# Dasch0/nenbody

Hardware: AMD Instinct MI355X
Metric: body-updates/sec (N x steps/s) at N=131072, all-pairs gravity + Euler step (higher is better)
Workload: dtype f32

## Files before the change

### nenbody_amd/csrc/nb_api.hip

```cpp
#include <hip/hip_runtime.h>
#include <dlfcn.h>

#include <cmath>
#include <cstdlib>
#include <algorithm>
#include <atomic>
#include <chrono>
#include <cstring>
#include <mutex>
#include <new>
#include <string>
#include <thread>
#include <vector>

#include "../../include/nenbody.h"
#include "../../include/nenbody_diag.h"
#include "nb_kernels.h"
#include "nb_eyes.h"
#include "nb_frame.h"
#define NB_SRGB_TABLE static const
#define NB_SRGB_WANT_DECODE
#include "nb_srgb_tables.h"
#undef NB_SRGB_WANT_DECODE
#undef NB_SRGB_TABLE

#define NB_EXPORT extern "C" __attribute__((visibility("default")))

namespace {

thread_local std::string g_tls_error = "";

constexpr uint32_t kTargetWaves = 16384;
constexpr uint32_t kMaxSlices = 64;

struct Knob {
    bool set = false;
    uint32_t v = 0;
    uint32_t or_else(uint32_t dflt) const { return set ? v : dflt; }
    bool on() const { return set && v != 0; }
};
struct DebugOverrides {
    Knob tile, fast_pairs_w, fast_pairs_np, fast_pairs_chunk, fast_ib, fast_groups, fast_waves, fast_slices, fast_no_share, strict_force_ieee, force_3d, strict_no_packed, strict_lanes, strict_unroll,
        strict_pc, strict_bc, strict_sl, fast_sl, fast_pairs, ring, ring_np, ring_ga, ring_wpb, ring_c4_own, ring_c4_rest, ring_cap, inst_device_libm, boids_slices, bc_spin_budget, bc_prio, boids_pc, boids_tile, boids_force, selftest_control, roctx, dropin_zero_copy, dropin_poll, dropin_poll_budget_us;
    uint32_t generation = 0;
};

Knob read_knob(const char *name)
{
    Knob k;
    const char *s = std::getenv(name);
    if (s && *s) {
        k.set = true;
        k.v = (uint32_t)std::strtoul(s, nullptr, 10);
    }
    return k;
}

std::atomic<const DebugOverrides *> g_overrides{nullptr};
std::atomic<bool> g_env_enabled{false};
std::atomic<bool> g_rccl_solo{false};
std::mutex g_overrides_mu;

const DebugOverrides *parse_overrides(uint32_t generation)
{
    DebugOverrides *d = new DebugOverrides();
    d->generation = generation;
    d->roctx = read_knob("NB_ROCTX");
    if (!g_env_enabled.load(std::memory_order_relaxed)) return d;
    d->tile = read_knob("NB_TILE");
    d->fast_ib = read_knob("NB_FAST_IB");
    d->fast_groups = read_knob("NB_FAST_GROUPS");
    d->fast_waves = read_knob("NB_FAST_WAVES");
    d->fast_slices = read_knob("NB_FAST_SLICES");
    d->fast_no_share = read_knob("NB_FAST_NO_SHARE");
    d->strict_force_ieee = read_knob("NB_STRICT_FORCE_IEEE");
    d->force_3d = read_knob("NB_FORCE_3D");
    d->strict_no_packed = read_knob("NB_STRICT_NO_PACKED");
    d->strict_lanes = read_knob("NB_STRICT_LANES");
    d->strict_unroll = read_knob("NB_STRICT_UNROLL");
    d->strict_pc = read_knob("NB_STRICT_PC");
    d->strict_bc = read_knob("NB_STRICT_BC");
    d->strict_sl = read_knob("NB_STRICT_SL");
    d->fast_sl = read_knob("NB_FAST_SL");
    d->fast_pairs = read_knob("NB_FAST_PAIRS");
    d->fast_pairs_w = read_knob("NB_FAST_PAIRS_W");
    d->fast_pairs_chunk = read_knob("NB_FAST_PAIRS_CHUNK");
    d->fast_pairs_np = read_knob("NB_FAST_PAIRS_NP");
    d->inst_device_libm = read_knob("NB_INST_DEVICE_LIBM");
    d->ring = read_knob("NB_RING");
    d->ring_np = read_knob("NB_RING_NP");
    d->ring_ga = read_knob("NB_RING_GA");
    d->ring_wpb = read_knob("NB_RING_WPB");
    d->ring_c4_own = read_knob("NB_RING_C4_OWN");
    d->ring_c4_rest = read_knob("NB_RING_C4_REST");
    d->ring_cap = read_knob("NB_RING_CAP");
    d->bc_spin_budget = read_knob("NB_BC_SPIN_BUDGET");
    d->bc_prio = read_knob("NB_BC_PRIO");
    d->boids_pc = read_knob("NB_BOIDS_PC");
    d->boids_tile = read_knob("NB_BOIDS_TILE");
    d->boids_force = read_knob("NB_BOIDS_FORCE");
    d->boids_slices = read_knob("NB_BOIDS_SLICES");
    d->dropin_zero_copy = read_knob("NB_DROPIN_ZERO_COPY");
    d->dropin_poll = read_knob("NB_DROPIN_POLL");
    d->dropin_poll_budget_us = read_knob("NB_DROPIN_POLL_BUDGET_US");
    d->selftest_control = read_knob("NB_SELFTEST_CONTROL");
    return d;
}

const DebugOverrides &overrides()
{
    const DebugOverrides *d = g_overrides.load(std::memory_order_acquire);
    if (d) return *d;
    std::lock_guard<std::mutex> lock(g_overrides_mu);
    d = g_overrides.load(std::memory_order_acquire);
    if (!d) {
        d = parse_overrides(1);
        g_overrides.store(d, std::memory_order_release);
    }
    return *d;
}

bool valid_tile(uint32_t t) { return t == 256 || t == 512 || t == 1024; }

struct Plan {
    uint32_t tile;
    uint32_t ib;
    uint32_t waves;
    uint32_t groups;
    uint32_t slices;
    uint32_t j_chunk;
    uint32_t lo_bits, hi_bits, force_ieee;
    int guard_a, guard_b, guard_g, guard_c;
    uint32_t force_3d;
    uint32_t unroll;
    uint32_t lanes;
    uint32_t pc;
    uint32_t no_packed;
    uint32_t bc;
    uint32_t pairs;
    uint32_t pairs_np;
    uint32_t pairs_chunk;
    uint32_t fsl;
    uint32_t sl;
    uint32_t spin_budget;
    uint32_t bc_prio;
    uint32_t n_total;
};

int floor_log2f(float x)
{
    int e;
    std::frexp(x, &e);
    return e - 1;
}

uint32_t fast_bodies_per_lane(uint32_t n_total, uint32_t count)
{
    const uint64_t pairs = (uint64_t)n_total * count;
    uint32_t ib = overrides().fast_ib.or_else(pairs >= (1ull << 31) ? 4u : pairs >= (1ull << 27) ? 2u : 1u);
    return (ib == 1 || ib == 2 || ib == 4) ? ib : 1u;
}

uint32_t fast_wave_form()
{
    const uint32_t w = overrides().fast_waves.or_else(8u);
    return (w == 1 || w == 4 || w == 8 || w == 16) ? w : 0u;
}

void fast_split(uint32_t n_fold, uint32_t count, uint32_t ib, uint32_t waves, uint32_t *tile, uint32_t *groups, uint32_t *slices,
                uint32_t *chunk)
{
    const DebugOverrides &dbg = overrides();
    if (waves && *tile == 1024u) *tile = 512u;
    if (waves && *tile == 512u && (ib == 1 || waves == 1)) *tile = 256u;
    const uint32_t bodies = waves ? 64u * ib : 256u * ib, chunk_waves = waves ? 1u : 4u;
    const uint32_t blocks = (count + bodies - 1u) / bodies;
    const uint32_t max_by_tiles = std::max(1u, (n_fold + *tile - 1u) / *tile);
    uint32_t split = (kTargetWaves + blocks * chunk_waves - 1u) / (blocks * chunk_waves);
    if (split > max_by_tiles) split = max_by_tiles;
    if (split < 1) split = 1;
    uint32_t g = waves ? waves : dbg.fast_groups.or_else(split >= 4u ? 4u : split >= 2u ? 2u : 1u);
    if (!waves && g != 1 && g != 2 && g != 4) g = 1;
    if (!waves && *tile == 1024u) g = 1;
    uint32_t sl = dbg.fast_slices.or_else((split + g - 1u) / g);
    if (sl > kMaxSlices) sl = kMaxSlices;
    if (sl < 1) sl = 1;
    uint32_t chunks = sl * g;
    if (chunks > max_by_tiles) chunks = max_by_tiles;
    uint32_t c = (std::max(n_fold, 1u) + chunks - 1u) / chunks;
    c = ((c + *tile - 1u) / *tile) * *tile;
    chunks = (std::max(n_fold, 1u) + c - 1u) / c;
    sl = (chunks + g - 1u) / g;
    *groups = g;
    *slices = sl;
    *chunk = c;
}

int make_plan(const nb_params &p, uint32_t n_total, uint32_t count, Plan *out, std::string *err)
{
    if (n_total == 0 || count == 0 || count > n_total) {
        *err = "nb: need 0 < count <= n_total";
        return NB_ERR_INVALID;
    }
    if (p.mode != NB_MODE_STRICT && p.mode != NB_MODE_FAST) {
        *err = "nb: params.mode must be NB_MODE_STRICT or NB_MODE_FAST";
        return NB_ERR_INVALID;
    }
    if (n_total > 0x80000000u) {
        *err = "nb: sets of more than 2^31 bodies are not supported";
        return NB_ERR_UNSUPPORTED;
    }
    const DebugOverrides &dbg = overrides();
    Plan pl{};
    pl.tile = p.tile;
    if (pl.tile == 0) pl.tile = dbg.tile.or_else((p.mode == NB_MODE_STRICT) ? 1024u : fast_wave_form() ? 256u : 512u);
    if (!valid_tile(pl.tile)) {
        *err = "nb: params.tile must be 0, 256, 512 or 1024";
        return NB_ERR_INVALID;
    }
    pl.ib = 1;
    pl.groups = 1;
    pl.slices = 1;
    pl.j_chunk = n_total;
    if (p.mode == NB_MODE_FAST) {
        pl.ib = fast_bodies_per_lane(n_total, count);
        pl.waves = fast_wave_form();
        fast_split(n_total, count, pl.ib, pl.waves, &pl.tile, &pl.groups, &pl.slices, &pl.j_chunk);
    }
    if (p.mode == NB_MODE_FAST) {
        const bool no_form_named = p.tile == 0 && !dbg.tile.set && !dbg.fast_waves.set && !dbg.fast_groups.set;
        pl.fsl = dbg.fast_sl.or_else((pl.waves == 8u && n_total >= 4096u && no_form_named) ? 1u : 0u);
        constexpr uint32_t kPairsMinN = 32768u;
        const bool pairs_ok = count == n_total && n_total % 256u == 0 && n_total <= 4194304u;
        uint32_t pnp = (n_total >= 98304u && n_total % 512u == 0) ? 4u : 2u;
        if (dbg.fast_pairs_np.set && (dbg.fast_pairs_np.v == 2 || (dbg.fast_pairs_np.v == 4 && n_total % 512u == 0))) pnp = dbg.fast_pairs_np.v;
        uint32_t pw = pnp == 4u ? (n_total >= 131072u ? 4u : 2u) : (n_total >= 131072u ? 8u : 4u);
        if (dbg.fast_pairs_w.set && (dbg.fast_pairs_w.v == 1 || dbg.fast_pairs_w.v == 2 || dbg.fast_pairs_w.v == 4 || (dbg.fast_pairs_w.v == 8 && pnp == 2u)))
            pw = dbg.fast_pairs_w.v;
        pl.pairs = (pairs_ok && dbg.fast_pairs.or_else((n_total >= kPairsMinN && no_form_named && !dbg.fast_sl.set && !dbg.fast_ib.set &&
                                                        !dbg.fast_slices.set) ? 1u : 0u)) ? pw : 0u;
        pl.pairs_np = pnp;
        pl.pairs_chunk = 0;
        if (pl.pairs && dbg.fast_pairs_chunk.on()) {
            const uint32_t super = 128u * pnp * pw;
            pl.pairs_chunk = std::max(super, dbg.fast_pairs_chunk.v / super * super);
        }
        if (pl.pairs) pl.fsl = 0;
        if (pl.fsl) {
            uint32_t tile = 256u;
            pl.waves = 8u;
            fast_split(n_total, count, pl.ib, pl.waves, &tile, &pl.groups, &pl.slices, &pl.j_chunk);
            pl.tile = tile;
        }
    }
    pl.force_ieee = 1;
    pl.lo_bits = 0x3f800000u;
    pl.hi_bits = 0x3f800000u;
    const float G = std::fabs(p.G);
    if (std::isfinite(p.G) && std::isfinite(p.bias) && G > 0.f && p.bias > 0.f) {
        const int g = floor_log2f(G), c = floor_log2f(p.bias);
        const int b = 20;
        const int dmax = std::max(2 * b + 4, c + 2);
        int a = std::max(-100 + 23 - g, -120 + 23 - g + dmax);
        const bool ok = g >= -100 && g <= 100 && c >= -100 && dmax <= 100 && (b + 2 + g - c) <= 120 && a <= b - 1;
        if (ok) {
            if (a < -120) a = -120;
            pl.lo_bits = (uint32_t)(a + 127) << 23;
            pl.hi_bits = (uint32_t)(b + 127) << 23;
            pl.force_ieee = 0;
            pl.guard_a = a;
            pl.guard_b = b;
            pl.guard_g = g;
            pl.guard_c = c;
        }
    }
    if (dbg.strict_force_ieee.on()) pl.force_ieee = 1;
    if (p.mode == NB_MODE_FAST) {
        const bool bias_ok = std::isfinite(p.bias) && p.bias >= 0x1p-60f && p.bias <= 0x1p60f;
        pl.force_ieee = (!bias_ok || dbg.fast_no_share.on()) ? 1u : 0u;
    }
    pl.force_3d = dbg.force_3d.on() ? 2u : 0u;
    pl.no_packed = dbg.strict_no_packed.on() ? 1u : 0u;
    constexpr uint32_t kChainMax = 57344u;
    pl.lanes = 1;
    if (count <= kChainMax)
        while (pl.lanes < 16 && (uint64_t)count * pl.lanes < 2048ull * 64ull) pl.lanes *= 2;
    pl.lanes = dbg.strict_lanes.or_else(pl.lanes);
    if (pl.lanes != 1 && pl.lanes != 2 && pl.lanes != 4 && pl.lanes != 8 && pl.lanes != 16) pl.lanes = 1;
    pl.unroll = dbg.strict_unroll.or_else(pl.lanes == 1 ? 8 : (pl.lanes == 16 ? 2 : 4));
    if (pl.lanes == 1 && pl.unroll != 4 && pl.unroll != 8 && pl.unroll != 16) pl.unroll = 8;
    if (pl.lanes > 1 && pl.unroll != 2 && pl.unroll != 4) pl.unroll = 4;
    if (pl.lanes == 16) pl.unroll = 2;
    if (p.mode == NB_MODE_STRICT && pl.lanes > 1 && pl.tile == 512) pl.tile = 1024;
    if (p.mode == NB_MODE_STRICT && pl.lanes > 1 && pl.tile == 1024 && pl.unroll == 2 && pl.lanes < 8) pl.unroll = 4;
    constexpr uint32_t kSmallSet = 1536u;
    pl.pc = dbg.strict_pc.or_else((count <= kChainMax && n_total >= kSmallSet) ? 14u : 0u);
    if (pl.pc == 1) pl.pc = 8;
    if (pl.pc != 0 && pl.pc != 8 && pl.pc != 14) pl.pc = 8;
    pl.n_total = n_total;
    pl.bc = dbg.strict_bc.or_else((count <= kChainMax && n_total >= kSmallSet && !dbg.strict_pc.set && !dbg.strict_lanes.set) ? 1u : 0u);
    pl.bc = (pl.bc && p.mode == NB_MODE_STRICT) ? 1u : 0u;
    pl.spin_budget = dbg.bc_spin_budget.or_else(0u);
    pl.bc_prio = dbg.bc_prio.or_else(1u) ? 1u : 0u;
    pl.sl = dbg.strict_sl.or_else((!pl.bc && !pl.pc && pl.lanes == 1 && p.tile == 0 && !dbg.tile.set && !dbg.strict_lanes.set &&
                                   !dbg.strict_pc.set && !dbg.strict_unroll.set && !dbg.strict_no_packed.set && n_total >= kSmallSet) ? 1u : 0u);
    pl.sl = (pl.sl && p.mode == NB_MODE_STRICT && !pl.bc) ? std::min(pl.sl, 3u) : 0u;
    *out = pl;
    return NB_OK;
}

size_t plan_scratch_bytes(const Plan &pl, uint32_t count)
{
    if (pl.bc || pl.sl) return nbk::strict_bc_scratch_bytes(pl.n_total);
    if (pl.pairs) return nbk::strict_bc_scratch_bytes(pl.n_total) + nbk::fast_pairs_scratch_floats(pl.n_total, pl.pairs, pl.pairs_np, pl.pairs_chunk) * sizeof(float);
    if (pl.fsl) return nbk::strict_bc_scratch_bytes(pl.n_total) + (pl.slices > 1 ? (size_t)pl.slices * count * sizeof(float4) : 0);
    return pl.slices > 1 ? (size_t)pl.slices * count * sizeof(float4) : 0;
}

int cached_plan(const nb_params &p, uint32_t n_total, uint32_t count, const Plan **out, std::string *err)
{
    struct Entry {
        bool valid = false;
        nb_params p{};
        uint32_t n_total = 0, count = 0, generation = 0;
        Plan pl{};
    };
    constexpr int kEntries = 4;
    thread_local Entry cache[kEntries];
    thread_local int next = 0;
    const uint32_t gen = overrides().generation;
    for (int i = 0; i < kEntries; ++i) {
        const Entry &e = cache[i];
        if (e.valid && e.n_total == n_total && e.count == count && e.generation == gen && std::memcmp(&e.p, &p, sizeof(p)) == 0) {
            *out = &e.pl;
            return NB_OK;
        }
    }
    Plan pl;
    int rc = make_plan(p, n_total, count, &pl, err);
    if (rc != NB_OK) return rc;
    Entry &e = cache[next];
    next = (next + 1) % kEntries;
    e.valid = true;
    e.p = p;
    e.n_total = n_total;
    e.count = count;
    e.generation = gen;
    e.pl = pl;
    *out = &e.pl;
    return NB_OK;
}

struct Roctx {
    int (*push)(const char *) = nullptr;
    int (*pop)() = nullptr;
};
const Roctx *roctx_api()
{
    if (!overrides().roctx.on()) return nullptr;
    static const Roctx *api = [] {
        Roctx *r = new Roctx();
        void *h = dlopen("librocprofiler-sdk-roctx.so.1", RTLD_NOW | RTLD_LOCAL);
        if (!h) h = dlopen("librocprofiler-sdk-roctx.so", RTLD_NOW | RTLD_LOCAL);
        if (!h) h = dlopen("libroctx64.so.4", RTLD_NOW | RTLD_LOCAL);
        if (!h) h = dlopen("libroctx64.so", RTLD_NOW | RTLD_LOCAL);
        if (h) {
            r->push = (int (*)(const char *))dlsym(h, "roctxRangePushA");
            r->pop = (int (*)())dlsym(h, "roctxRangePop");
        }
        return (const Roctx *)r;
    }();
    return (api->push && api->pop) ? api : nullptr;
}
struct RoctxRange {
    const Roctx *api;
    explicit RoctxRange(const char *name) : api(roctx_api())
    {
        if (api) (void)api->push(name);
    }
    ~RoctxRange()
    {
        if (api) (void)api->pop();
    }
    RoctxRange(const RoctxRange &) = delete;
    RoctxRange &operator=(const RoctxRange &) = delete;
};

constexpr int kMaxDevices = 64;
uint32_t *g_status_word[kMaxDevices] = {};
std::mutex g_status_mu;

int device_status_word(uint32_t **out, std::string *err)
{
    int dev = 0;
    hipError_t e = hipGetDevice(&dev);
    if (e != hipSuccess || dev < 0 || dev >= kMaxDevices) {
        *err = std::string("nb: hipGetDevice failed: ") + hipGetErrorString(e);
        return NB_ERR_HIP;
    }
    std::lock_guard<std::mutex> lock(g_status_mu);
    if (!g_status_word[dev]) {
        uint32_t *w = nullptr;
        e = hipMalloc((void **)&w, 64);
        if (e == hipSuccess) e = hipMemset(w, 0, 64);
        if (e != hipSuccess) {
            *err = std::string("nb: allocating the device status word failed: ") + hipGetErrorString(e);
            return e == hipErrorOutOfMemory ? NB_ERR_ALLOC : NB_ERR_HIP;
        }
        g_status_word[dev] = w;
    }
    *out = g_status_word[dev];
    return NB_OK;
}

int check_status_word(uint32_t *w, std::string *err)
{
    if (!w) return NB_OK;
    uint32_t v = 0;
    hipError_t e = hipMemcpy(&v, w, sizeof(v), hipMemcpyDeviceToHost);
    if (e != hipSuccess) {
        *err = std::string("nb: reading the device status word failed: ") + hipGetErrorString(e);
        return NB_ERR_HIP;
    }
    if (v == 0u) return NB_OK;
    (void)hipMemset(w, 0, sizeof(v));
    *err = "nb: a STRICT block-chain workgroup gave up waiting for its turn (its outputs are NaN): the state is invalid; "
           "upload it again";
    return NB_ERR_STATE;
}

int check_device_status(std::string *err)
{
    int dev = 0;
    if (hipGetDevice(&dev) != hipSuccess || dev < 0 || dev >= kMaxDevices) return NB_OK;
    uint32_t *w;
    {
        std::lock_guard<std::mutex> lock(g_status_mu);
        w = g_status_word[dev];
    }
    return check_status_word(w, err);
}

struct StatusWord {
    uint32_t *w = nullptr;
    bool dirty = false;
};

int status_word_for_launch(StatusWord *sw, std::string *err)
{
    if (!sw->w) {
        hipError_t e = hipMalloc((void **)&sw->w, 64);
        if (e == hipSuccess) e = hipMemset(sw->w, 0, 64);
        if (e != hipSuccess) {
            *err = std::string("nb: allocating the status word failed: ") + hipGetErrorString(e);
            return e == hipErrorOutOfMemory ? NB_ERR_ALLOC : NB_ERR_HIP;
        }
    }
    sw->dirty = true;
    return NB_OK;
}

int check_status(StatusWord *sw, std::string *err)
{
    if (!sw->dirty) return NB_OK;
    sw->dirty = false;
    return check_status_word(sw->w, err);
}

int launch_step_planned(const nb_params &p, const Plan &pl, uint32_t n_total, uint32_t first, uint32_t count,
                        const void *pos_in, void *pos_out, void *vel, void *scratch, hipStream_t stream, std::string *err,
                        StatusWord *sw = nullptr)
{
    nbk::StepArgs a{};
    a.pos_in = (const float4 *)pos_in;
    a.pos_out = (float4 *)pos_out;
    a.vel = (float4 *)vel;
    a.partial = (float4 *)scratch;
    a.n_total = n_total;
    a.first = first;
    a.count = count;
    a.dt = p.dt;
    a.G = p.G;
    a.bias = p.bias;
    a.lo_bits = pl.lo_bits;
    a.hi_bits = pl.hi_bits;
    a.force_ieee = pl.force_ieee;
    a.force_3d = pl.force_3d;
    a.j_chunk = pl.j_chunk;
    a.no_packed = pl.no_packed;
    a.spin_budget = pl.spin_budget;
    a.bc_prio = pl.bc_prio;
    a.j_count = n_total;
    a.j_base = 0;
    a.hole_lo = 0xffffffffu;
    a.hole_len = 0;
    uint32_t *status = nullptr;
    if (p.mode == NB_MODE_STRICT && pl.bc) {
        int rc = sw ? status_word_for_launch(sw, err) : device_status_word(&status, err);
        if (rc != NB_OK) return rc;
        if (sw) status = sw->w;
    }
    hipError_t e = (p.mode == NB_MODE_STRICT) ? (pl.bc   ? nbk::launch_strict_bc(a, scratch, status, stream)
                                                 : pl.sl ? nbk::launch_strict_sl(a, pl.sl - 1u, scratch, stream)
                                                 : pl.pc ? nbk::launch_strict_pc(a, pl.pc, stream)
                                                       : nbk::launch_strict(a, pl.tile, pl.unroll, pl.lanes, stream))
                                              : pl.pairs ? nbk::launch_fast_pairs(a, pl.pairs, pl.pairs_np, pl.pairs_chunk, scratch, stream)
                                              : pl.fsl   ? nbk::launch_fast_sl(a, pl.ib, pl.slices, scratch, stream)
                                              : pl.waves ? nbk::launch_fast_wave(a, pl.tile, pl.ib, pl.waves, pl.slices, stream)
                                                         : nbk::launch_fast(a, pl.tile, pl.ib, pl.groups, pl.slices, stream);
    if (e == hipErrorNotSupported) {
        *err = "nb: this launch shape is one of the legacy forms (NB_STRICT_PC / NB_STRICT_LANES / NB_STRICT_UNROLL / NB_STRICT_SL=2,3 / "
               "NB_FAST_WAVES / NB_FAST_GROUPS / NB_FAST_PAIRS_W): this library was built without them (make -C nenbody_amd/csrc legacy "
               "builds libnenbody_hip_legacy.so, which holds every form)";
        return NB_ERR_UNSUPPORTED;
    }
    if (e != hipSuccess) {
        *err = std::string("nb: kernel launch failed: ") + hipGetErrorString(e);
        return NB_ERR_HIP;
    }
    return NB_OK;
}

int check_device(std::string *err)
{
    static std::atomic<bool> seen{false};
    if (seen.load(std::memory_order_relaxed)) return NB_OK;
    int n = 0;
    hipError_t e = hipGetDeviceCount(&n);
    if (e != hipSuccess || n <= 0) {
        (void)hipGetLastError();
        *err = std::string("nb: no HIP device available (") + (e == hipSuccess ? "0 devices" : hipGetErrorString(e)) +
               "); this library has no CPU path";
        return NB_ERR_NO_DEVICE;
    }
    seen.store(true, std::memory_order_relaxed);
    return NB_OK;
}

float sqrt_threshold(float r)
{
// ... 1718 lines not shown
```

### nenbody_amd/csrc/nb_nbody_sym.inc

```
constexpr int pr_block(int np) { return 128 * np; }

template <int kNP>
struct PrState {
    v2f xi[kNP], yi[kNP], zi[kNP];
    v2f ax[kNP], ay[kNP], az[kNP];
};

__device__ __forceinline__ float pr_rotate_sub(float acc, float t)
{
    return __int_as_float(__builtin_amdgcn_update_dpp(0, __float_as_int(acc), 0x134 , 0xf, 0xf, false)) - t;
}
__device__ __forceinline__ float pr_rotate(float acc)
{
    return __int_as_float(__builtin_amdgcn_update_dpp(0, __float_as_int(acc), 0x134, 0xf, 0xf, false));
}

template <bool PLANAR, bool SHARED, int K, int kNP>
__device__ __forceinline__ void pr_steps(PrState<kNP> &s, const float (&bx)[K], const float (&by)[K], const float (&bz)[K], v2f bias2, float &sx,
                                         float &sy, float &sz)
{
    v2f dx[K][kNP], dy[K][kNP], dz[K][kNP], r2[K][kNP], inv[K][kNP], tx[K], ty[K], tz[K];
#define NBK_ROW _Pragma("unroll") for (int k = 0; k < K; ++k) _Pragma("unroll") for (int b = 0; b < kNP; ++b)
#define NBK_ROWK _Pragma("unroll") for (int k = 0; k < K; ++k)
    NBK_ROW dx[k][b] = v2f{bx[k], bx[k]} - s.xi[b];
// ... 1 lines not shown
    NBK_ROW r2[k][b] = __builtin_elementwise_fma(dx[k][b], dx[k][b], bias2);
    if (!PLANAR) {
        NBK_ROW dz[k][b] = v2f{bz[k], bz[k]} - s.zi[b];
    }
    NBK_ROW r2[k][b] = __builtin_elementwise_fma(dy[k][b], dy[k][b], r2[k][b]);
    if (!PLANAR) {
        NBK_ROW r2[k][b] = __builtin_elementwise_fma(dz[k][b], dz[k][b], r2[k][b]);
    }
    if (SHARED) {
        float p[K][kNP], rp[K][kNP];
        NBK_ROW p[k][b] = r2[k][b].x * r2[k][b].y;
        NBK_ROW rp[k][b] = __builtin_amdgcn_rcpf(p[k][b]);
        NBK_ROW inv[k][b] = v2f{rp[k][b], rp[k][b]} * v2f{r2[k][b].y, r2[k][b].x};
    } else {
        NBK_ROW inv[k][b] = (v2f{__builtin_amdgcn_rcpf(r2[k][b].x), __builtin_amdgcn_rcpf(r2[k][b].y)});
    }
    NBK_ROWK tx[k] = dx[k][0] * inv[k][0];
    NBK_ROWK ty[k] = dy[k][0] * inv[k][0];
    if (!PLANAR) {
        NBK_ROWK tz[k] = dz[k][0] * inv[k][0];
    }
#pragma unroll
    for (int b = 1; b < kNP; ++b) {
        NBK_ROWK tx[k] = __builtin_elementwise_fma(dx[k][b], inv[k][b], tx[k]);
        NBK_ROWK ty[k] = __builtin_elementwise_fma(dy[k][b], inv[k][b], ty[k]);
        if (!PLANAR) {
            NBK_ROWK tz[k] = __builtin_elementwise_fma(dz[k][b], inv[k][b], tz[k]);
        }
    }
#if defined(NB_EXP_NOPIN)
#elif defined(NB_EXP_PIN_SUMS)
    NBK_ROWK {
        _Pragma("unroll") for (int b = 0; b < kNP; ++b) {
            asm volatile("" : "+v"(s.ax[b]), "+v"(s.ay[b]));
            if (!PLANAR) asm volatile("" : "+v"(s.az[b]));
        }
    }
#else
    NBK_ROWK {
        asm volatile("" : "+v"(tx[k]), "+v"(ty[k]));
        if (!PLANAR) asm volatile("" : "+v"(tz[k]));
        _Pragma("unroll") for (int b = 0; b < kNP; ++b) {
            asm volatile("" : "+v"(s.ax[b]), "+v"(s.ay[b]));
            if (!PLANAR) asm volatile("" : "+v"(s.az[b]));
        }
    }
#endif
    NBK_ROWK {
        _Pragma("unroll") for (int b = 0; b < kNP; ++b) s.ax[b] = __builtin_elementwise_fma(dx[k][b], inv[k][b], s.ax[b]);
        _Pragma("unroll") for (int b = 0; b < kNP; ++b) s.ay[b] = __builtin_elementwise_fma(dy[k][b], inv[k][b], s.ay[b]);
        if (!PLANAR) {
            _Pragma("unroll") for (int b = 0; b < kNP; ++b) s.az[b] = __builtin_elementwise_fma(dz[k][b], inv[k][b], s.az[b]);
        }
    }
    NBK_ROWK {
        sx = pr_rotate_sub(sx, tx[k].x);
        sy = pr_rotate_sub(sy, ty[k].x);
        if (!PLANAR) sz = pr_rotate_sub(sz, tz[k].x);
        sx = sx - tx[k].y;
        sy = sy - ty[k].y;
        if (!PLANAR) sz = sz - tz[k].y;
    }
#undef NBK_ROW
#undef NBK_ROWK
}

constexpr int kPrK = 1;
constexpr int kPrTrip = 32;
template <bool PLANAR, bool SHARED, int kNP>
__device__ __forceinline__ void pr_sweep(PrState<kNP> &s, const float2 *pl, const float *plz, float bias, float &bx, float &by, float &bz)
{
    constexpr int K = kPrK, T = kPrTrip;
    const v2f bias2 = {bias, bias};
    float sx = 0.f, sy = 0.f, sz = 0.f;
    float2 cur[K];
    float curz[K];
#pragma unroll
    for (int k = 0; k < K; ++k) cur[k] = pl[k], curz[k] = PLANAR ? 0.f : plz[k];
#pragma unroll 1
    for (int s0 = 0; s0 < 64; s0 += T) {
#pragma unroll
        for (int u = 0; u < T; u += K) {
            float2 nxt[K];
            float nxtz[K];
#pragma unroll
            for (int k = 0; k < K; ++k) nxt[k] = pl[s0 + u + K + k], nxtz[k] = PLANAR ? 0.f : plz[s0 + u + K + k];
            float qx[K], qy[K], qz[K];
#pragma unroll
            for (int k = 0; k < K; ++k) qx[k] = cur[k].x, qy[k] = cur[k].y, qz[k] = curz[k];
            pr_steps<PLANAR, SHARED, K, kNP>(s, qx, qy, qz, bias2, sx, sy, sz);
#pragma unroll
            for (int k = 0; k < K; ++k) cur[k] = nxt[k], curz[k] = nxtz[k];
        }
    }
    bx = pr_rotate(sx);
    by = pr_rotate(sy);
    bz = PLANAR ? 0.f : pr_rotate(sz);
}

struct PrTile {
    float *rows_a, *rows_b;
    uint32_t ra, la, a0;
    uint32_t rb, lb, b0;
    uint32_t p0, q0, np, nq, rect;
};

#if defined(NB_EXP_OCC4)
#define NB_PR_OCC __attribute__((amdgpu_waves_per_eu(4, 4)))
#else
#define NB_PR_OCC
#endif
template <int kPrW, int kNP>
__global__ __launch_bounds__(64 * kPrW) NB_PR_OCC void step_fast_pairs_kernel(StepArgs a, const uint32_t *__restrict__ flags, uint32_t generation,
                                                                    const float *__restrict__ px, const float *__restrict__ py,
                                                                    const float *__restrict__ pz, PrTile tl)
{
    constexpr int kPrBlock = pr_block(kNP), kPrSuper = kPrBlock * kPrW;
    __shared__ float2 slab[kPrW][128];
    __shared__ float slabz[kPrW][128];
    __shared__ float accb[3][kPrSuper];
    const ClockStamp stamp0 = clock_begin(a.stamps);
    uint32_t pl_, ql_;
    if (tl.rect) {
        pl_ = blockIdx.x / tl.nq;
        ql_ = blockIdx.x - pl_ * tl.nq;
    } else {
        uint32_t rem = blockIdx.x, len = tl.np - 1u;
        pl_ = 0;
        while (rem >= len) {
            rem -= len;
            ++pl_;
            --len;
        }
        ql_ = pl_ + 1u + rem;
    }
    const uint32_t P = tl.p0 + pl_, Q = tl.q0 + ql_;
    const int w = __builtin_amdgcn_readfirstlane((int)threadIdx.x >> 6);
    const int lane = (int)threadIdx.x & 63;
    const uint32_t n = a.n_total;
    const uint32_t nblocks = n / (uint32_t)kPrBlock;
    const uint32_t ia = P * (uint32_t)kPrW + (uint32_t)w;
    const bool have_a = ia < nblocks;
    const uint32_t f = ((uint32_t)__builtin_amdgcn_readfirstlane(flags[kBcFlagWordIeee]) == generation ? kFlagIeee : 0u) |
                       ((uint32_t)__builtin_amdgcn_readfirstlane(flags[kBcFlagWordNonPlanar]) == generation ? kFlagNonPlanar : 0u) | a.force_3d;
    const bool share = ((f | a.force_ieee) & kFlagIeee) == 0u;
    const bool planar = (f & kFlagNonPlanar) == 0u;

    PrState<kNP> s;
    {
        const uint32_t i0 = (have_a ? ia : 0u) * (uint32_t)kPrBlock + (uint32_t)lane;
#pragma unroll
        for (int b = 0; b < kNP; ++b) {
            s.xi[b] = v2f{px[i0 + 128u * b], px[i0 + 128u * b + 64u]};
            s.yi[b] = v2f{py[i0 + 128u * b], py[i0 + 128u * b + 64u]};
            s.zi[b] = planar ? v2f{0.f, 0.f} : v2f{pz[i0 + 128u * b], pz[i0 + 128u * b + 64u]};
            s.ax[b] = s.ay[b] = s.az[b] = v2f{0.f, 0.f};
        }
    }
    for (int k = (int)threadIdx.x; k < 3 * kPrSuper; k += 64 * kPrW) (&accb[0][0])[k] = 0.f;
    __syncthreads();

    struct Rec {
        float x, y, z;
    };
    auto block_of = [&](int p) { return Q * (uint32_t)kPrW + (uint32_t)((w + p) & (kPrW - 1)); };
    auto fetch = [&](int p, int t) {
        Rec r = {0.f, 0.f, 0.f};
        const uint32_t jb = block_of(p);
        if (have_a && p < kPrW && jb < nblocks) {
            const uint32_t j = jb * (uint32_t)kPrBlock + (uint32_t)(t * 64 + lane);
            r.x = px[j];
            r.y = py[j];
            if (!planar) r.z = pz[j];
        }
        return r;
    };
    Rec r_next = fetch(0, 0);
    for (int p = 0; p < kPrW; ++p) {
        const int qb = (w + p) & (kPrW - 1);
        const bool have_b = have_a && block_of(p) < nblocks;
#pragma unroll 1
        for (int t = 0; t < kPrBlock / 64; ++t) {
            const Rec r = r_next;
            r_next = (t + 1 < kPrBlock / 64) ? fetch(p, t + 1) : fetch(p + 1, 0);
            if (!have_b) continue;
            __builtin_amdgcn_wave_barrier();
            slab[w][lane] = slab[w][64 + lane] = make_float2(r.x, r.y);
            if (!planar) slabz[w][lane] = slabz[w][64 + lane] = r.z;
            __builtin_amdgcn_wave_barrier();
            float bx, by, bz;
            if (planar && share)
                pr_sweep<true, true, kNP>(s, &slab[w][lane], &slabz[w][lane], a.bias, bx, by, bz);
            else if (planar)
                pr_sweep<true, false, kNP>(s, &slab[w][lane], &slabz[w][lane], a.bias, bx, by, bz);
            else if (share)
                pr_sweep<false, true, kNP>(s, &slab[w][lane], &slabz[w][lane], a.bias, bx, by, bz);
            else
                pr_sweep<false, false, kNP>(s, &slab[w][lane], &slabz[w][lane], a.bias, bx, by, bz);
            const int idx = qb * kPrBlock + t * 64 + lane;
            accb[0][idx] = accb[0][idx] + bx;
            accb[1][idx] = accb[1][idx] + by;
            if (!planar) accb[2][idx] = accb[2][idx] + bz;
        }
        __syncthreads();
    }
    if (have_a) {
        const size_t plane = (size_t)tl.ra * tl.la;
        float *const row = tl.rows_a + (size_t)ql_ * tl.la + ((size_t)ia * kPrBlock - tl.a0) + (uint32_t)lane;
#pragma unroll
        for (int b = 0; b < kNP; ++b) {
            row[128 * b] = s.ax[b].x, row[128 * b + 64] = s.ax[b].y;
            row[plane + 128 * b] = s.ay[b].x, row[plane + 128 * b + 64] = s.ay[b].y;
            if (!planar) row[2 * plane + 128 * b] = s.az[b].x, row[2 * plane + 128 * b + 64] = s.az[b].y;
        }
    }
    const uint32_t q_lo = Q * (uint32_t)kPrSuper;
    const size_t planeb = (size_t)tl.rb * tl.lb;
    float *const rowq = tl.rows_b + (size_t)pl_ * tl.lb + (q_lo - tl.b0);
    for (int k = (int)threadIdx.x; k < kPrSuper; k += 64 * kPrW) {
        if (q_lo + (uint32_t)k >= n) break;
        rowq[k] = accb[0][k];
        rowq[planeb + k] = accb[1][k];
        if (!planar) rowq[2 * planeb + k] = accb[2][k];
    }
    clock_end(a.stamps, stamp0);
}

template <int kPrW, int kNP>
__global__ __launch_bounds__(64 * kPrW) void pairs_diag_kernel(StepArgs a, const uint32_t *__restrict__ flags, uint32_t generation,
                                                               const float *__restrict__ px, const float *__restrict__ py,
                                                               const float *__restrict__ pz, PrTile tl)
{
    constexpr int IB = 2 * kNP;
    constexpr int kPrBlock = pr_block(kNP), kPrSuper = kPrBlock * kPrW;
    __shared__ float part[kPrW > 1 ? kPrW - 1 : 1][3][kPrBlock];
    const int w = __builtin_amdgcn_readfirstlane((int)threadIdx.x >> 6);
    const int lane = (int)threadIdx.x & 63;
    const uint32_t n = a.n_total;
    const uint32_t block = tl.p0 * (uint32_t)kPrW + blockIdx.x;
    const uint32_t base = block * (uint32_t)kPrBlock + (uint32_t)lane;
    const uint32_t P = block / (uint32_t)kPrW;
    FslState<IB> s;
#pragma unroll
    for (int b = 0; b < IB; ++b) {
        const uint32_t l = base + (uint32_t)(b * 64);
        const float x = px[l], y = py[l], z = pz[l];
        s.xi[b] = v2f{x, x};
        s.yi[b] = v2f{y, y};
        s.zi[b] = v2f{z, z};
        s.ax[b] = s.ay[b] = s.az[b] = v2f{0.f, 0.f};
    }
    const uint32_t f = ((uint32_t)__builtin_amdgcn_readfirstlane(flags[kBcFlagWordIeee]) == generation ? kFlagIeee : 0u) |
                       ((uint32_t)__builtin_amdgcn_readfirstlane(flags[kBcFlagWordNonPlanar]) == generation ? kFlagNonPlanar : 0u) | a.force_3d;
    const bool share = ((f | a.force_ieee) & kFlagIeee) == 0u;
    const bool planar = (f & kFlagNonPlanar) == 0u;
    const uint32_t lo = P * (uint32_t)kPrSuper + (uint32_t)w * (uint32_t)kPrBlock;
    const uint32_t j_lo = lo < n ? lo : n, j_hi = lo + (uint32_t)kPrBlock < n ? lo + (uint32_t)kPrBlock : n;
    if (planar && share)
        fsl_range<true, true, IB>(s, px, py, pz, j_lo, j_hi, a.bias);
    else if (planar)
        fsl_range<true, false, IB>(s, px, py, pz, j_lo, j_hi, a.bias);
    else if (share)
        fsl_range<false, true, IB>(s, px, py, pz, j_lo, j_hi, a.bias);
    else
        fsl_range<false, false, IB>(s, px, py, pz, j_lo, j_hi, a.bias);
    float ax[IB], ay[IB], az[IB];
#pragma unroll
    for (int b = 0; b < IB; ++b) {
        ax[b] = s.ax[b].x + s.ax[b].y;
        ay[b] = s.ay[b].x + s.ay[b].y;
        az[b] = s.az[b].x + s.az[b].y;
    }
    if (kPrW > 1) {
        if (w > 0) {
#pragma unroll
            for (int b = 0; b < IB; ++b) {
                part[w - 1][0][b * 64 + lane] = ax[b];
                part[w - 1][1][b * 64 + lane] = ay[b];
                part[w - 1][2][b * 64 + lane] = az[b];
            }
        }
        __syncthreads();
        if (w > 0) return;
#pragma unroll
        for (int g = 1; g < kPrW; ++g) {
#pragma unroll
            for (int b = 0; b < IB; ++b) {
                ax[b] = ax[b] + part[g - 1][0][b * 64 + lane];
                ay[b] = ay[b] + part[g - 1][1][b * 64 + lane];
                az[b] = az[b] + part[g - 1][2][b * 64 + lane];
            }
        }
    }
    const size_t plane = (size_t)tl.ra * tl.la;
    float *const row = tl.rows_a + (size_t)(P - tl.p0) * tl.la + (base - tl.a0);
#pragma unroll
    for (int b = 0; b < IB; ++b) {
        row[64 * b] = ax[b];
        row[plane + 64 * b] = ay[b];
        if (!planar) row[2 * plane + 64 * b] = az[b];
    }
}

__global__ __launch_bounds__(256) void pairs_integrate_kernel(StepArgs a, const uint32_t *__restrict__ flags, uint32_t generation,
                                                              const float *__restrict__ rows, uint32_t ns)
{
    const uint32_t l = blockIdx.x * 256u + threadIdx.x;
    if (l >= a.count) return;
    const bool planar = (flags[kBcFlagWordNonPlanar] != generation) && !a.force_3d;
    const size_t plane = (size_t)ns * a.n_total;
    float sx = 0.f, sy = 0.f, sz = 0.f;
    const float *r = rows + l;
    for (uint32_t k = 0; k < ns; ++k, r += a.n_total) {
        sx = sx + r[0];
        sy = sy + r[plane];
        if (!planar) sz = sz + r[2 * plane];
    }
    float4 p = a.pos_in[l];
    float4 v = a.vel[l];
    integrate(p, v, sx * a.G, sy * a.G, sz * a.G, a.dt);
    a.vel[l] = v;
    a.pos_out[l] = p;
}

__global__ __launch_bounds__(256) void pairs_accumulate_kernel(const uint32_t *__restrict__ flags, uint32_t generation, uint32_t force_3d,
                                                               float *__restrict__ acc, uint32_t n, const float *__restrict__ rows, uint32_t r_,
                                                               uint32_t len, uint32_t first, uint32_t fresh)
{
    const uint32_t l = blockIdx.x * 256u + threadIdx.x;
    if (l >= len || first + l >= n) return;
    const bool planar = (flags[kBcFlagWordNonPlanar] != generation) && !force_3d;
    const size_t plane = (size_t)r_ * len;
    float *const dst = acc + first + l;
    float sx = fresh ? 0.f : dst[0], sy = fresh ? 0.f : dst[n], sz = (fresh || planar) ? 0.f : dst[2 * (size_t)n];
    const float *r = rows + l;
    for (uint32_t k = 0; k < r_; ++k, r += len) {
        sx = sx + r[0];
        sy = sy + r[plane];
        if (!planar) sz = sz + r[2 * plane];
    }
    dst[0] = sx;
    dst[n] = sy;
    if (!planar) dst[2 * (size_t)n] = sz;
}
__global__ __launch_bounds__(256) void pairs_finish_kernel(StepArgs a, const uint32_t *__restrict__ flags, uint32_t generation,
                                                           const float *__restrict__ acc)
{
    const uint32_t l = blockIdx.x * 256u + threadIdx.x;
    if (l >= a.count) return;
    const bool planar = (flags[kBcFlagWordNonPlanar] != generation) && !a.force_3d;
    const float sx = acc[l], sy = acc[a.n_total + l], sz = planar ? 0.f : acc[2 * (size_t)a.n_total + l];
    float4 p = a.pos_in[l];
    float4 v = a.vel[l];
    integrate(p, v, sx * a.G, sy * a.G, sz * a.G, a.dt);
    a.vel[l] = v;
    a.pos_out[l] = p;
}

constexpr uint32_t kPrOneTileMax = 262144u;
constexpr uint32_t kPrChunk = 131072u;
uint32_t fast_pairs_chunk(uint32_t n_total, uint32_t chunk) { return chunk ? chunk : n_total <= kPrOneTileMax ? n_total : kPrChunk; }
size_t fast_pairs_scratch_floats(uint32_t n_total, uint32_t w, uint32_t np, uint32_t chunk)
{
    const uint32_t c = fast_pairs_chunk(n_total, chunk), super = (uint32_t)pr_block((int)np) * w;
    const size_t rows = (size_t)3 * ((c + super - 1u) / super) * c;
    return c >= n_total ? rows : (size_t)3 * n_total + 2 * rows;
}

template <int W, int NP>
static hipError_t launch_fast_pairs_w(const StepArgs &a, uint32_t chunk, const uint32_t *flags, uint32_t generation, const float *px,
                                      const float *py, const float *pz, float *scratch, hipStream_t s)
{
    constexpr uint32_t kPrBlock = (uint32_t)pr_block(NP);
    const uint32_t super = kPrBlock * W, n = a.n_total;
    auto tile = [&](uint32_t a0, uint32_t la, uint32_t b0, uint32_t lb, float *rows_a, float *rows_b) -> hipError_t {
        PrTile tl{};
        tl.p0 = a0 / super, tl.np = (la + super - 1u) / super, tl.a0 = a0, tl.la = la;
        tl.q0 = b0 / super, tl.nq = (lb + super - 1u) / super, tl.b0 = b0, tl.lb = lb;
        tl.rect = a0 != b0;
        tl.rows_a = rows_a, tl.rows_b = rows_b;
        tl.ra = tl.rect ? tl.nq : tl.np, tl.rb = tl.np;
        if (!tl.rect) {
            hipLaunchKernelGGL((pairs_diag_kernel<W, NP>), dim3(la / kPrBlock), dim3(64 * W), 0, s, a, flags, generation, px, py, pz, tl);
            if (tl.np > 1u)
                hipLaunchKernelGGL((step_fast_pairs_kernel<W, NP>), dim3(tl.np * (tl.np - 1u) / 2u), dim3(64 * W), 0, s, a, flags, generation, px, py, pz, tl);
        } else {
            hipLaunchKernelGGL((step_fast_pairs_kernel<W, NP>), dim3(tl.np * tl.nq), dim3(64 * W), 0, s, a, flags, generation, px, py, pz, tl);
        }
        return hipGetLastError();
    };
    if (chunk >= n) {
        hipError_t e = tile(0, n, 0, n, scratch, scratch);
        if (e != hipSuccess) return e;
        hipLaunchKernelGGL(pairs_integrate_kernel, dim3((a.count + 255u) / 256u), dim3(256), 0, s, a, flags, generation, scratch, (n + super - 1u) / super);
        return hipGetLastError();
    }
    float *const acc = scratch;
    const size_t rows_floats = (size_t)3 * ((chunk + super - 1u) / super) * chunk;
    float *const rows_a = acc + (size_t)3 * n, *const rows_b = rows_a + rows_floats;
    auto accumulate = [&](const float *rows, uint32_t r_, uint32_t len, uint32_t first, bool fresh) {
        hipLaunchKernelGGL(pairs_accumulate_kernel, dim3((len + 255u) / 256u), dim3(256), 0, s, flags, generation, a.force_3d, acc, n, rows, r_, len, first,
                           fresh ? 1u : 0u);
    };
    for (uint32_t a0 = 0; a0 < n; a0 += chunk) {
        const uint32_t la = n - a0 < chunk ? n - a0 : chunk, npa = (la + super - 1u) / super;
        hipError_t e = tile(a0, la, a0, la, rows_a, rows_a);
        if (e != hipSuccess) return e;
        accumulate(rows_a, npa, la, a0, a0 == 0);
        for (uint32_t b0 = a0 + chunk; b0 < n; b0 += chunk) {
            const uint32_t lb = n - b0 < chunk ? n - b0 : chunk, npb = (lb + super - 1u) / super;
            e = tile(a0, la, b0, lb, rows_a, rows_b);
            if (e != hipSuccess) return e;
            accumulate(rows_a, npb, la, a0, false);
            accumulate(rows_b, npa, lb, b0, a0 == 0);
        }
    }
    hipLaunchKernelGGL(pairs_finish_kernel, dim3((a.count + 255u) / 256u), dim3(256), 0, s, a, flags, generation, acc);
    return hipGetLastError();
}
hipError_t launch_fast_pairs_kernels(const StepArgs &a, uint32_t w, uint32_t np, uint32_t chunk, const uint32_t *flags, uint32_t generation,
                                     const float *px, const float *py, const float *pz, float *scratch, hipStream_t s)
{
    chunk = fast_pairs_chunk(a.n_total, chunk);
#define NBK_PAIRS(W_, NP_) \
    if (w == W_ && np == NP_) return launch_fast_pairs_w<W_, NP_>(a, chunk, flags, generation, px, py, pz, scratch, s)
    NBK_PAIRS(4, 4);
    NBK_PAIRS(2, 4);
    NBK_PAIRS(8, 2);
    NBK_PAIRS(4, 2);
#ifdef NB_LEGACY_FORMS
    NBK_PAIRS(2, 2);
    NBK_PAIRS(1, 2);
    NBK_PAIRS(1, 4);
#endif
#undef NBK_PAIRS
    return hipErrorNotSupported;
}
uint32_t fast_pairs_rows(uint32_t n_total, uint32_t w, uint32_t np)
{
    const uint32_t super = (uint32_t)pr_block((int)np) * w;
    return (n_total + super - 1u) / super;
}
```

Before: 23.86 million.

## Add NP=8 pairs form with remapped diagonal pass and batched row reduction

Adds a symmetric-pairs configuration with eight i-bodies per lane (W=2, NP=8), selected by default for N>=131072 divisible by 1024. The diagonal kernel stays capped at NP=4 and takes more waves, so it covers the same superblock. Separately, the row-combine loops in the integrate and accumulate kernels now issue eight strided loads before summing, to expose memory-level parallelism. More bodies per lane raises register reuse of each j-body but increases register pressure, which can lower occupancy or cause spills.

```diff
diff --git a/nenbody_amd/csrc/nb_api.hip b/nenbody_amd/csrc/nb_api.hip
--- a/nenbody_amd/csrc/nb_api.hip
+++ b/nenbody_amd/csrc/nb_api.hip
@@ -232,10 +232,13 @@
         pl.fsl = dbg.fast_sl.or_else((pl.waves == 8u && n_total >= 4096u && no_form_named) ? 1u : 0u);
         constexpr uint32_t kPairsMinN = 32768u;
         const bool pairs_ok = count == n_total && n_total % 256u == 0 && n_total <= 4194304u;
-        uint32_t pnp = (n_total >= 98304u && n_total % 512u == 0) ? 4u : 2u;
-        if (dbg.fast_pairs_np.set && (dbg.fast_pairs_np.v == 2 || (dbg.fast_pairs_np.v == 4 && n_total % 512u == 0))) pnp = dbg.fast_pairs_np.v;
-        uint32_t pw = pnp == 4u ? (n_total >= 131072u ? 4u : 2u) : (n_total >= 131072u ? 8u : 4u);
-        if (dbg.fast_pairs_w.set && (dbg.fast_pairs_w.v == 1 || dbg.fast_pairs_w.v == 2 || dbg.fast_pairs_w.v == 4 || (dbg.fast_pairs_w.v == 8 && pnp == 2u)))
+        uint32_t pnp = (n_total >= 131072u && n_total % 1024u == 0) ? 8u : (n_total >= 98304u && n_total % 512u == 0) ? 4u : 2u;
+        if (dbg.fast_pairs_np.set && (dbg.fast_pairs_np.v == 2 || (dbg.fast_pairs_np.v == 4 && n_total % 512u == 0) ||
+                                      (dbg.fast_pairs_np.v == 8 && n_total % 1024u == 0)))
+            pnp = dbg.fast_pairs_np.v;
+        uint32_t pw = pnp == 8u ? 2u : pnp == 4u ? (n_total >= 131072u ? 4u : 2u) : (n_total >= 131072u ? 8u : 4u);
+        if (dbg.fast_pairs_w.set && (dbg.fast_pairs_w.v == 1 || dbg.fast_pairs_w.v == 2 || (dbg.fast_pairs_w.v == 4 && pnp != 8u) ||
+                                     (dbg.fast_pairs_w.v == 8 && pnp == 2u)))
             pw = dbg.fast_pairs_w.v;
         pl.pairs = (pairs_ok && dbg.fast_pairs.or_else((n_total >= kPairsMinN && no_form_named && !dbg.fast_sl.set && !dbg.fast_ib.set &&
                                                         !dbg.fast_slices.set) ? 1u : 0u)) ? pw : 0u;
diff --git a/nenbody_amd/csrc/nb_nbody_sym.inc b/nenbody_amd/csrc/nb_nbody_sym.inc
--- a/nenbody_amd/csrc/nb_nbody_sym.inc
+++ b/nenbody_amd/csrc/nb_nbody_sym.inc
@@ -327,20 +327,49 @@
     }
 }
 
-__global__ __launch_bounds__(256) void pairs_integrate_kernel(StepArgs a, const uint32_t *__restrict__ flags, uint32_t generation,
-                                                              const float *__restrict__ rows, uint32_t ns)
-{
-    const uint32_t l = blockIdx.x * 256u + threadIdx.x;
+constexpr int kPrRowsAhead = 8;
+__device__ __forceinline__ void pr_add_rows(const float *r, size_t stride, size_t plane, uint32_t rows, bool planar, float &sx, float &sy, float &sz)
+{
+    uint32_t k = 0;
+    for (; k + (uint32_t)kPrRowsAhead <= rows; k += (uint32_t)kPrRowsAhead, r += (size_t)kPrRowsAhead * stride) {
+        float x[kPrRowsAhead], y[kPrRowsAhead], z[kPrRowsAhead];
+#pragma unroll
+        for (int u = 0; u < kPrRowsAhead; ++u) x[u] = r[(size_t)u * stride];
+#pragma unroll
+        for (int u = 0; u < kPrRowsAhead; ++u) y[u] = r[plane + (size_t)u * stride];
+        if (!planar) {
+#pragma unroll
+            for (int u = 0; u < kPrRowsAhead; ++u) z[u] = r[2 * plane + (size_t)u * stride];
+        }
+#pragma unroll
+        for (int u = 0; u < kPrRowsAhead; ++u) sx = sx + x[u];
+#pragma unroll
+        for (int u = 0; u < kPrRowsAhead; ++u) sy = sy + y[u];
+        if (!planar) {
+#pragma unroll
+            for (int u = 0; u < kPrRowsAhead; ++u) sz = sz + z[u];
+        }
+    }
+    for (; k < rows; ++k, r += stride) {
+        sx = sx + r[0];
+        sy = sy + r[plane];
+        if (!planar) sz = sz + r[2 * plane];
+    }
+}
+
+#if !defined(NB_EXP_COMBINE_WG)
+#define NB_EXP_COMBINE_WG 256
+#endif
+constexpr uint32_t kPrCombineWg = NB_EXP_COMBINE_WG;
+__global__ __launch_bounds__(kPrCombineWg) void pairs_integrate_kernel(StepArgs a, const uint32_t *__restrict__ flags, uint32_t generation,
+                                                                       const float *__restrict__ rows, uint32_t ns)
+{
+    const uint32_t l = blockIdx.x * kPrCombineWg + threadIdx.x;
     if (l >= a.count) return;
     const bool planar = (flags[kBcFlagWordNonPlanar] != generation) && !a.force_3d;
     const size_t plane = (size_t)ns * a.n_total;
     float sx = 0.f, sy = 0.f, sz = 0.f;
-    const float *r = rows + l;
-    for (uint32_t k = 0; k < ns; ++k, r += a.n_total) {
-        sx = sx + r[0];
-        sy = sy + r[plane];
-        if (!planar) sz = sz + r[2 * plane];
-    }
+    pr_add_rows(rows + l, a.n_total, plane, ns, planar, sx, sy, sz);
     float4 p = a.pos_in[l];
     float4 v = a.vel[l];
     integrate(p, v, sx * a.G, sy * a.G, sz * a.G, a.dt);
@@ -358,12 +387,7 @@
     const size_t plane = (size_t)r_ * len;
     float *const dst = acc + first + l;
     float sx = fresh ? 0.f : dst[0], sy = fresh ? 0.f : dst[n], sz = (fresh || planar) ? 0.f : dst[2 * (size_t)n];
-    const float *r = rows + l;
-    for (uint32_t k = 0; k < r_; ++k, r += len) {
-        sx = sx + r[0];
-        sy = sy + r[plane];
-        if (!planar) sz = sz + r[2 * plane];
-    }
+    pr_add_rows(rows + l, len, plane, r_, planar, sx, sy, sz);
     dst[0] = sx;
     dst[n] = sy;
     if (!planar) dst[2 * (size_t)n] = sz;
@@ -393,10 +417,16 @@
 }
 
 template <int W, int NP>
+struct PrDiagShape {
+    static constexpr int kNP = NP > 4 ? 4 : NP, kW = W * (NP / kNP);
+    static_assert(pr_block(kNP) * kW == pr_block(NP) * W, "the diagonal pass and the sweep must share the superblock");
+};
+template <int W, int NP>
 static hipError_t launch_fast_pairs_w(const StepArgs &a, uint32_t chunk, const uint32_t *flags, uint32_t generation, const float *px,
                                       const float *py, const float *pz, float *scratch, hipStream_t s)
 {
     constexpr uint32_t kPrBlock = (uint32_t)pr_block(NP);
+    constexpr int DW = PrDiagShape<W, NP>::kW, DNP = PrDiagShape<W, NP>::kNP;
     const uint32_t super = kPrBlock * W, n = a.n_total;
     auto tile = [&](uint32_t a0, uint32_t la, uint32_t b0, uint32_t lb, float *rows_a, float *rows_b) -> hipError_t {
         PrTile tl{};
@@ -406,7 +436,7 @@
         tl.rows_a = rows_a, tl.rows_b = rows_b;
         tl.ra = tl.rect ? tl.nq : tl.np, tl.rb = tl.np;
         if (!tl.rect) {
-            hipLaunchKernelGGL((pairs_diag_kernel<W, NP>), dim3(la / kPrBlock), dim3(64 * W), 0, s, a, flags, generation, px, py, pz, tl);
+            hipLaunchKernelGGL((pairs_diag_kernel<DW, DNP>), dim3(la / (uint32_t)pr_block(DNP)), dim3(64 * DW), 0, s, a, flags, generation, px, py, pz, tl);
             if (tl.np > 1u)
                 hipLaunchKernelGGL((step_fast_pairs_kernel<W, NP>), dim3(tl.np * (tl.np - 1u) / 2u), dim3(64 * W), 0, s, a, flags, generation, px, py, pz, tl);
         } else {
@@ -417,7 +447,7 @@
     if (chunk >= n) {
         hipError_t e = tile(0, n, 0, n, scratch, scratch);
         if (e != hipSuccess) return e;
-        hipLaunchKernelGGL(pairs_integrate_kernel, dim3((a.count + 255u) / 256u), dim3(256), 0, s, a, flags, generation, scratch, (n + super - 1u) / super);
+        hipLaunchKernelGGL(pairs_integrate_kernel, dim3((a.count + kPrCombineWg - 1u) / kPrCombineWg), dim3(kPrCombineWg), 0, s, a, flags, generation, scratch, (n + super - 1u) / super);
         return hipGetLastError();
     }
     float *const acc = scratch;
@@ -449,6 +479,7 @@
     chunk = fast_pairs_chunk(a.n_total, chunk);
 #define NBK_PAIRS(W_, NP_) \
     if (w == W_ && np == NP_) return launch_fast_pairs_w<W_, NP_>(a, chunk, flags, generation, px, py, pz, scratch, s)
+    NBK_PAIRS(2, 8);
     NBK_PAIRS(4, 4);
     NBK_PAIRS(2, 4);
     NBK_PAIRS(8, 2);
@@ -457,6 +488,7 @@
     NBK_PAIRS(2, 2);
     NBK_PAIRS(1, 2);
     NBK_PAIRS(1, 4);
+    NBK_PAIRS(1, 8);
 #endif
 #undef NBK_PAIRS
     return hipErrorNotSupported;
```

Measured after the change: 23.84 million. About the same (-0.1%).
